# AhauBioinformatics/IDDGCN

Measured on AMD Instinct MI355X. Metric: adjacency edges/s per IDDGCN training step (pos fwd + neg fwd + bwd + Adam), higher is better.
Workload: dtype f32

## Files before the change

### iddgcn_amd/csrc/iddgcn_hip.hip

```cpp
#include <hip/hip_runtime.h>
#include <stdint.h>

#include <type_traits>

#include "../../include/iddgcn.h"

typedef float f32x4 __attribute__((ext_vector_type(4)));
typedef float f32x16 __attribute__((ext_vector_type(16)));
typedef _Float16 f16x4 __attribute__((ext_vector_type(4)));
typedef _Float16 f16x8 __attribute__((ext_vector_type(8)));
typedef __bf16 bf16x8 __attribute__((ext_vector_type(8)));
typedef __bf16 bf16x4 __attribute__((ext_vector_type(4)));
typedef short s16x4 __attribute__((ext_vector_type(4)));
typedef unsigned int u32x2 __attribute__((ext_vector_type(2)));
typedef unsigned int u32x4 __attribute__((ext_vector_type(4)));

#define MAX_R 8
#define EPS_BCE 1e-7f

namespace {

__device__ __forceinline__ float sigmoidf_(float x) { return 1.0f / (1.0f + expf(-x)); }
__device__ __forceinline__ float sigmoid_fast(float x) { return __builtin_amdgcn_rcpf(1.0f + __expf(-x)); }

// ... 1555 lines not shown
            __builtin_amdgcn_sched_barrier(0);
        }
        __builtin_amdgcn_sched_barrier(0);
        {
            v4s16 ta[2][2], tb[2][4][2];
#pragma unroll
            for (int s = 0; s < 2; ++s) {
                const int ra = 16 * s + 8 * (lane >> 5) + xs, rq = ra + 4;
                tr_read_asm(ta[s][0], xb + ra * XPT + 16 * ((4 * wb + colq) ^ stn_sw(ra)) + cb);
                tr_read_asm(ta[s][1], xb + rq * XPT + 16 * ((4 * wb + colq) ^ stn_sw(rq)) + cb);
#pragma unroll
                for (int j = 0; j < 4; ++j) {
                    const int blk = cbase + j;
                    tr_read_asm(tb[s][j][0], dob + ra * DPT + 16 * ((4 * blk + colq) ^ stn_sw(ra)) + cb);
                    tr_read_asm(tb[s][j][1], dob + rq * DPT + 16 * ((4 * blk + colq) ^ stn_sw(rq)) + cb);
                }
            }
            asm volatile("s_waitcnt lgkmcnt(0)"
                         : "+v"(ta[0][0]), "+v"(ta[0][1]), "+v"(ta[1][0]), "+v"(ta[1][1]), "+v"(tb[0][0][0]),
                           "+v"(tb[0][0][1]), "+v"(tb[0][1][0]), "+v"(tb[0][1][1]), "+v"(tb[0][2][0]),
                           "+v"(tb[0][2][1]), "+v"(tb[0][3][0]), "+v"(tb[0][3][1]), "+v"(tb[1][0][0]),
                           "+v"(tb[1][0][1]), "+v"(tb[1][1][0]), "+v"(tb[1][1][1]), "+v"(tb[1][2][0]),
                           "+v"(tb[1][2][1]), "+v"(tb[1][3][0]), "+v"(tb[1][3][1])::"memory");
#pragma unroll
            for (int s = 0; s < 2; ++s) {
                const bf16x8 a = __builtin_bit_cast(bf16x8, __builtin_shufflevector(ta[s][0], ta[s][1], 0, 1, 2, 3, 4, 5, 6, 7));
#pragma unroll
                for (int j = 0; j < 4; ++j)
                    tacc[j] = __builtin_amdgcn_mfma_f32_32x32x16_bf16(
                        a, __builtin_bit_cast(bf16x8, __builtin_shufflevector(tb[s][j][0], tb[s][j][1], 0, 1, 2, 3, 4, 5, 6, 7)),
                        tacc[j], 0, 0, 0);
            }
        }
        __builtin_amdgcn_sched_barrier(0);
    };
    auto epilogue = [&](long long t, int bb, const f32x4 (&sacc)[2]) __attribute__((always_inline)) -> int {
        const char* xb = lds + bb * BUF + DOB;
        const long long row0 = t * TR;
        const long long left = M - row0;
        const unsigned nbytes = (unsigned)((left < TR ? left : TR) * D * 2);
        const __amdgpu_buffer_rsrc_t rc =
            __builtin_amdgcn_make_buffer_rsrc(reinterpret_cast<char*>(X) + row0 * D * 2, (short)0, nbytes, 0x00020000);
        const int xc = (2 * wave + (g >> 1)) ^ swi;
#pragma unroll
        for (int rb = 0; rb < 2; ++rb) {
            const int r = 16 * rb + i16;
            const f32x4 x = bf4_to_f32(*reinterpret_cast<const bf16x4*>(xb + r * XPT + 16 * xc + 8 * (g & 1)));
            f32x4 v = sacc[rb];
#pragma unroll
            for (int q = 0; q < 4; ++q) v[q] = v[q] * (x[q] * (1.0f - x[q]));
            __builtin_amdgcn_raw_buffer_store_b64(__builtin_bit_cast(u32x2, f32_to_bf4(v)), rc, (r * D + c0 + 4 * g) * 2,
                                                  0, 0);
        }
        return 2;
    };

    if (t_beg < t_end) {
        int dc[PD], sc[PD];
#pragma unroll
        for (int k = 0; k < PD; ++k) {
            dc[k] = t_beg + k < t_end ? stage(t_beg + k, k) : 0;
            sc[k] = 0;
        }
        int younger = 0;
#pragma unroll
        for (int k = 1; k < PD; ++k) younger += dc[k];
        wait_vm(younger);
        asm volatile("s_waitcnt lgkmcnt(0)" ::: "memory");
        __syncthreads();
        f32x4 sacc[2];
        int b = 0;
        for (long long t = t_beg; t < t_end; ++t) {
            const int it = (int)(t - t_beg);
            const int slot = it % PD;
            dc[slot] = t + PD < t_end ? stage(t + PD, (b + PD) % NBUF) : 0;
            mfma_tile(b, sacc);
            sc[slot] = epilogue(t, b, sacc);
            int y = sc[(it + 1) % PD];
#pragma unroll
            for (int j = 2; j <= PD; ++j) {
                const int s2 = (it + j) % PD;
                y += dc[s2] + sc[s2];
            }
            wait_vm(y);
            asm volatile("s_waitcnt lgkmcnt(0)" ::: "memory");
            __builtin_amdgcn_s_barrier();
            asm volatile("" ::: "memory");
            b = (b + 1) % NBUF;
        }
    }
    float* out = slab + (long long)range * D * D;
    const int i = lane & 31, h = lane >> 5;
#pragma unroll
    for (int j = 0; j < 4; ++j)
#pragma unroll
        for (int k = 0; k < 16; ++k) {
            const int row = 128 * half + 32 * wb + (k & 3) + 8 * (k >> 2) + 4 * h;
            out[row * D + 32 * (cbase + j) + i] = tacc[j][k];
        }
}

__device__ __forceinline__ void split3(float x, __bf16& b0, __bf16& b1, __bf16& b2) {
    b0 = (__bf16)x;
    const float r1 = x - (float)b0;
    b1 = (__bf16)r1;
    b2 = (__bf16)(r1 - (float)b1);
}
typedef float f32x2v __attribute__((ext_vector_type(2)));
typedef __bf16 bf16x2v __attribute__((ext_vector_type(2)));
__device__ __forceinline__ unsigned cvt_pk_bf16(float a, float b) {
    return __builtin_bit_cast(unsigned, __builtin_convertvector(f32x2v{a, b}, bf16x2v));
}
__device__ __forceinline__ void split3x2(float x0, float x1, unsigned& p0, unsigned& p1, unsigned& p2) {
    p0 = cvt_pk_bf16(x0, x1);
    const float r0 = x0 - __builtin_bit_cast(float, p0 << 16);
    const float r1 = x1 - __builtin_bit_cast(float, p0 & 0xffff0000u);
    p1 = cvt_pk_bf16(r0, r1);
    const float s0 = r0 - __builtin_bit_cast(float, p1 << 16);
    const float s1 = r1 - __builtin_bit_cast(float, p1 & 0xffff0000u);
    p2 = cvt_pk_bf16(s0, s1);
}
__device__ __forceinline__ void split3x4(const f32x4& v, bf16x4& p0, bf16x4& p1, bf16x4& p2) {
    unsigned a0, b0, c0, a1, b1, c1;
    split3x2(v[0], v[1], a0, b0, c0);
    split3x2(v[2], v[3], a1, b1, c1);
    const u32x2 a = {a0, a1}, b = {b0, b1}, c = {c0, c1};
    p0 = __builtin_bit_cast(bf16x4, a);
    p1 = __builtin_bit_cast(bf16x4, b);
    p2 = __builtin_bit_cast(bf16x4, c);
}
__device__ __forceinline__ void planes_from3(const f32x4& x, char* row, int lane) {
    bf16x4 p0, p1, p2;
    split3x4(x, p0, p1, p2);
    *reinterpret_cast<bf16x4*>(row + lane * 8) = p0;
    *reinterpret_cast<bf16x4*>(row + 512 + lane * 8) = p1;
    *reinterpret_cast<bf16x4*>(row + 1024 + lane * 8) = p2;
}
__device__ __forceinline__ void row_to_planes3(char* row, int lane) {
    planes_from3(ld4(reinterpret_cast<const float*>(row) + lane * 4), row, lane);
}

__device__ __forceinline__ unsigned lds_u32(const void* p) {
    return (unsigned)(uintptr_t)(__attribute__((address_space(3))) const char*)p;
}
namespace rb3 {
constexpr int D = 256, NW = 8, TR = 32, CWG = 128, CWV = 16;
constexpr int PITCH = 1568;
constexpr int ABYTES = TR * PITCH;
constexpr int RPW = TR / NW;
constexpr int SLAB = TR * CWV;
}
__device__ __forceinline__ int slab16_off(int slot, int g) { return slot * 16 + 4 * (g ^ ((-(slot >> 2)) & 3)); }

template <int NV, bool AUX, bool BC = false>
__global__ __launch_bounds__(512) void rowgemm256_b3_kernel(RowGemmP p, int n_ranges) {
    using namespace rb3;
    static_assert(NV >= 0 && NV <= 2 && !(NV > 0 && AUX), "b3: gathered forward (NV = R = 1, 2), sigma' backward, plain");
    static_assert(!BC || NV == 0, "BC: one broadcast V row per relation (R <= 2), e.g. dz W_a^T");
    constexpr int NSL = NV + (AUX ? 1 : 0);
    constexpr int WF = NSL * SLAB + 64 + 64 + 32;
    constexpr int LDSB = 2 * ABYTES + NW * WF * 4;
    static_assert(LDSB <= 160 * 1024, "LDS budget");
    __shared__ __attribute__((aligned(16))) char lds[LDSB];
    const int lane = threadIdx.x & 63;
    const int wave = __builtin_amdgcn_readfirstlane(threadIdx.x >> 6);
    const int i = lane & 15, g = lane >> 4;
    const int bx = blockIdx.x;
    const int half = (bx >> 3) & 1;
    const int range = ((bx >> 4) << 3) | (bx & 7);
    if (range >= n_ranges) return;
    const int c0 = half * CWG + wave * CWV;
    float* slabw = reinterpret_cast<float*>(lds + 2 * ABYTES) + wave * WF;
    float* coefw = slabw + NSL * SLAB;
    int* idxw = reinterpret_cast<int*>(coefw + 64);
    int* cmpw = idxw + 64;

    const long long ntiles = ((long long)p.M + TR - 1) / TR;
    const long long t_beg = (long long)range * p.tiles_per_block;
    long long t_end = t_beg + p.tiles_per_block;
    if (t_end > ntiles) t_end = ntiles;
    if (t_beg >= t_end) return;
    const long long Mlast = (long long)p.M - 1;
    auto clampe = [&](long long e) __attribute__((always_inline)) { return e > Mlast ? Mlast : e; };

    bf16x8 w0[8], w1[8], w2[8];
#pragma unroll
    for (int q = 0; q < 8; ++q)
#pragma unroll
        for (int e = 0; e < 8; ++e) {
            const int k = 32 * q + 8 * g + e;
            const float wv = p.b_trans ? p.B[(c0 + i) * D + k] : p.B[k * D + c0 + i];
            __bf16 a, b, c;
            split3(wv, a, b, c);
            w0[q][e] = a;
            w1[q][e] = b;
            w2[q][e] = c;
        }

    f32x4 vb[2] = {f32x4{0.f, 0.f, 0.f, 0.f}, f32x4{0.f, 0.f, 0.f, 0.f}};
    if constexpr (BC) {
#pragma unroll
        for (int r = 0; r < 2; ++r)
            if (r < p.R) vb[r] = ld4(p.V + r * p.v_rel_stride + c0 + 4 * g);
    }
    auto dma_idx = [&](long long t) __attribute__((always_inline)) -> int {
        if (NV == 0 || !p.v_idx || t >= t_end) return 0;
        const int* src = p.v_idx + (lane < 32 ? clampe(t * TR + lane) : 0);
        __builtin_amdgcn_global_load_lds((gbl_vptr)src, (lds_vptr)idxw, 4, 0, 0);
        return 1;
    };
    auto dma_A = [&](long long t, int bb) __attribute__((always_inline)) -> int {
        if (t >= t_end) return 0;
#pragma unroll
        for (int j = 0; j < RPW; ++j) {
            const int r = wave * RPW + j;
            const float* src = p.A + clampe(t * TR + r) * D + lane * 4;
            __builtin_amdgcn_global_load_lds((gbl_vptr)src, (lds_vptr)(lds + bb * ABYTES + r * PITCH), 16, 0, 0);
        }
        return RPW;
    };
    auto convert = [&](int bb) __attribute__((always_inline)) {
#pragma unroll
        for (int j = 0; j < RPW; ++j) row_to_planes3(lds + bb * ABYTES + (wave * RPW + j) * PITCH, lane);
    };
    int vs0 = 0, vs1 = 0;
    auto dma_slabs = [&](long long t) __attribute__((always_inline)) -> int {
        int n = 0;
        if constexpr (NV > 0) {
            int vi = 0;
            bool start = false;
            if (lane < 32) {
                const long long e = clampe(t * TR + lane);
                vi = p.v_idx ? idxw[lane] : (int)e;
                const int prev = p.v_idx ? idxw[lane > 0 ? lane - 1 : 0] : (int)e - 1;
                start = lane == 0 || vi != prev;
            }
            const unsigned long long m = __ballot(start);
            const int u = __popcll(m);
            vs0 = __popcll(m & ((2ull << i) - 1)) - 1;
            vs1 = __popcll(m & ((2ull << (16 + i)) - 1)) - 1;
            if (start) cmpw[__popcll(m & ((2ull << lane) - 1)) - 1] = vi;
            asm volatile("s_waitcnt lgkmcnt(0)" ::: "memory");
            for (int kb = 0; kb < u; kb += 16) {
                const int slot = kb + (lane >> 2);
                const int gg = (lane & 3) ^ ((-(slot >> 2)) & 3);
                const long long v = cmpw[slot < u ? slot : u - 1];
#pragma unroll
                for (int r = 0; r < NV; ++r) {
                    const float* src = p.V + r * p.v_rel_stride + v * D + c0 + gg * 4;
                    __builtin_amdgcn_global_load_lds((gbl_vptr)src, (lds_vptr)(slabw + r * SLAB + kb * 16), 16, 0, 0);
                }
                n += NV;
            }
            const long long last = (long long)p.M * NV - 1;
            long long ci = t * TR * NV + lane;
            if (ci > last) ci = last;
            __builtin_amdgcn_global_load_lds((gbl_vptr)(p.coef + ci), (lds_vptr)coefw, 4, 0, 0);
            n += 1;
        }
        if constexpr (BC) {
            const long long last = (long long)p.M * p.R - 1;
            long long ci = t * TR * p.R + lane;
            if (ci > last) ci = last;
            __builtin_amdgcn_global_load_lds((gbl_vptr)(p.coef + ci), (lds_vptr)coefw, 4, 0, 0);
            n += 1;
        }
        if constexpr (AUX) {
#pragma unroll
            for (int k = 0; k < 2; ++k) {
                const int slot = 16 * k + (lane >> 2);
                const int gg = (lane & 3) ^ ((-(slot >> 2)) & 3);
                const float* src = p.aux + clampe(t * TR + slot) * D + c0 + gg * 4;
                __builtin_amdgcn_global_load_lds((gbl_vptr)src, (lds_vptr)(slabw + NV * SLAB + k * 256), 16, 0, 0);
            }
            n += 2;
        }
        return n;
    };
    auto epilogue = [&](long long t, const f32x4 (&acc)[2]) __attribute__((always_inline)) -> int {
        const long long row0 = t * TR;
        const long long left = (long long)p.M - row0;
        const unsigned nbytes = (unsigned)((left < TR ? left : TR) * D * 4);
        const __amdgpu_buffer_rsrc_t rc =
            __builtin_amdgcn_make_buffer_rsrc(reinterpret_cast<char*>(p.C) + row0 * D * 4, (short)0, nbytes, 0x00020000);
#pragma unroll
        for (int rh = 0; rh < 2; ++rh) {
            const int row = 16 * rh + i;
            f32x4 v = acc[rh];
            if constexpr (NV > 0) {
                const int vs = rh ? vs1 : vs0;
#pragma unroll
                for (int r = 0; r < NV; ++r) {
                    const float cf = coefw[row * NV + r];
                    const f32x4 s = ld4(slabw + r * SLAB + slab16_off(vs, g));
#pragma unroll
                    for (int q = 0; q < 4; ++q) v[q] = fmaf(cf, s[q], v[q]);
                }
            }
            if constexpr (BC) {
#pragma unroll
                for (int r = 0; r < 2; ++r) {
                    if (r >= p.R) break;
                    const float cf = coefw[row * p.R + r];
#pragma unroll
                    for (int q = 0; q < 4; ++q) v[q] = fmaf(cf, vb[r][q], v[q]);
                }
            }
            if (AUX && p.accumulate) {
                v += ld4(slabw + NV * SLAB + slab16_off(row, g));
            } else if (p.act == IDDGCN_ACT_SIGMOID) {
#pragma unroll
                for (int q = 0; q < 4; ++q) v[q] = sigmoid_fast(v[q]);
            } else if (AUX && p.act == IDDGCN_ACT_DSIGMOID) {
                const f32x4 x = ld4(slabw + NV * SLAB + slab16_off(row, g));
#pragma unroll
                for (int q = 0; q < 4; ++q) v[q] = v[q] * (x[q] * (1.0f - x[q]));
            }
            __builtin_amdgcn_raw_buffer_store_b128(v, rc, (row * D + c0 + 4 * g) * 4, 0, 0);
        }
        return 2;
    };
    auto mfma_tile = [&](int bb, f32x4 (&acc)[2]) __attribute__((always_inline)) {
        f32x4 hi0 = {0.f, 0.f, 0.f, 0.f}, lo0 = hi0, hi1 = hi0, lo1 = hi0;
        const unsigned ab = (unsigned)(uintptr_t)(__attribute__((address_space(3))) char*)(lds + bb * ABYTES) +
                            i * PITCH + 16 * g;
        u32x4 fx[2][3], fy[2][3];
        asm volatile("s_waitcnt lgkmcnt(0)" ::: "memory");
#define B3_LOADQ(Q, S)                                                                                    \
        asm volatile("ds_read_b128 %0, %6 offset:%7\n\tds_read_b128 %1, %6 offset:%8\n\t"                 \
                     "ds_read_b128 %2, %6 offset:%9\n\tds_read_b128 %3, %6 offset:%10\n\t"                \
                     "ds_read_b128 %4, %6 offset:%11\n\tds_read_b128 %5, %6 offset:%12"                   \
                     : "=&v"(fx[S][0]), "=&v"(fx[S][1]), "=&v"(fx[S][2]), "=&v"(fy[S][0]), "=&v"(fy[S][1]),     \
                       "=&v"(fy[S][2])                                                                   \
                     : "v"(ab), "i"(64 * (Q)), "i"(64 * (Q) + 512), "i"(64 * (Q) + 1024),                \
                       "i"(64 * (Q) + 16 * PITCH), "i"(64 * (Q) + 16 * PITCH + 512),                      \
                       "i"(64 * (Q) + 16 * PITCH + 1024)                                                 \
                     : "memory")
        B3_LOADQ(0, 0);
#pragma unroll
        for (int q = 0; q < 8; ++q) {
            const int S = q & 1;
            if (q + 1 < 8) {
                switch (q) {
                    case 0: B3_LOADQ(1, 1); break;
                    case 1: B3_LOADQ(2, 0); break;
                    case 2: B3_LOADQ(3, 1); break;
                    case 3: B3_LOADQ(4, 0); break;
                    case 4: B3_LOADQ(5, 1); break;
                    case 5: B3_LOADQ(6, 0); break;
                    default: B3_LOADQ(7, 1); break;
                }
                asm volatile("s_waitcnt lgkmcnt(6)"
                             : "+v"(fx[S][0]), "+v"(fx[S][1]), "+v"(fx[S][2]), "+v"(fy[S][0]), "+v"(fy[S][1]),
                               "+v"(fy[S][2])::"memory");
            } else {
                asm volatile("s_waitcnt lgkmcnt(0)"
                             : "+v"(fx[S][0]), "+v"(fx[S][1]), "+v"(fx[S][2]), "+v"(fy[S][0]), "+v"(fy[S][1]),
                               "+v"(fy[S][2])::"memory");
            }
            const bf16x8 x0 = __builtin_bit_cast(bf16x8, fx[S][0]), x1 = __builtin_bit_cast(bf16x8, fx[S][1]),
                         x2 = __builtin_bit_cast(bf16x8, fx[S][2]);
            const bf16x8 y0 = __builtin_bit_cast(bf16x8, fy[S][0]), y1 = __builtin_bit_cast(bf16x8, fy[S][1]),
                         y2 = __builtin_bit_cast(bf16x8, fy[S][2]);
            lo0 = __builtin_amdgcn_mfma_f32_16x16x32_bf16(w0[q], x2, lo0, 0, 0, 0);
            lo1 = __builtin_amdgcn_mfma_f32_16x16x32_bf16(w0[q], y2, lo1, 0, 0, 0);
            lo0 = __builtin_amdgcn_mfma_f32_16x16x32_bf16(w2[q], x0, lo0, 0, 0, 0);
            lo1 = __builtin_amdgcn_mfma_f32_16x16x32_bf16(w2[q], y0, lo1, 0, 0, 0);
            lo0 = __builtin_amdgcn_mfma_f32_16x16x32_bf16(w1[q], x1, lo0, 0, 0, 0);
            lo1 = __builtin_amdgcn_mfma_f32_16x16x32_bf16(w1[q], y1, lo1, 0, 0, 0);
            lo0 = __builtin_amdgcn_mfma_f32_16x16x32_bf16(w0[q], x1, lo0, 0, 0, 0);
            lo1 = __builtin_amdgcn_mfma_f32_16x16x32_bf16(w0[q], y1, lo1, 0, 0, 0);
            lo0 = __builtin_amdgcn_mfma_f32_16x16x32_bf16(w1[q], x0, lo0, 0, 0, 0);
            lo1 = __builtin_amdgcn_mfma_f32_16x16x32_bf16(w1[q], y0, lo1, 0, 0, 0);
            hi0 = __builtin_amdgcn_mfma_f32_16x16x32_bf16(w0[q], x0, hi0, 0, 0, 0);
            hi1 = __builtin_amdgcn_mfma_f32_16x16x32_bf16(w0[q], y0, hi1, 0, 0, 0);
        }
#undef B3_LOADQ
        acc[0] = hi0 + lo0;
        acc[1] = hi1 + lo1;
    };

    dma_idx(t_beg);
    asm volatile("s_waitcnt vmcnt(0)" ::: "memory");
    dma_A(t_beg, 0);
    dma_slabs(t_beg);
    asm volatile("s_waitcnt vmcnt(0) lgkmcnt(0)" ::: "memory");
    convert(0);
    dma_idx(t_beg + 1);
    asm volatile("s_waitcnt vmcnt(0) lgkmcnt(0)" ::: "memory");
    __syncthreads();

#define B3_MAIN_LOOP(LATE)                                                                           \
    {                                                                                                \
        f32x4 acc[2];                                                                                \
        int b = 0;                                                                                   \
        for (long long t = t_beg; t < t_end; ++t) {                                                  \
            const bool more = t + 1 < t_end;                                                         \
            const int nA = dma_A(t + 1, b ^ 1);                                                      \
            int after_A = 0;                                            \
            if (LATE && t > t_beg) {                                                                 \
                wait_vm(nA);                                                 \
                after_A += epilogue(t - 1, acc);                                                     \
                asm volatile("s_waitcnt lgkmcnt(0)" ::: "memory");                                   \
                after_A += dma_slabs(t);                                                             \
                asm volatile("s_waitcnt lgkmcnt(0)" ::: "memory");                                   \
                after_A += dma_idx(t + 1);                                                           \
            }                                                                                        \
            mfma_tile(b, acc);                                                                       \
            if (LATE) {                                                                              \
                if (more) {                                                                          \
                    wait_vm(after_A);                                                                \
                    convert(b ^ 1);                                                                  \
                }                                                                                    \
            } else {                                                                                 \
                wait_vm(nA);                                                 \
                after_A += epilogue(t, acc);                                                         \
                if (more) {                                                                          \
                    wait_vm(after_A);                                                    \
                    convert(b ^ 1);                                                                  \
                    asm volatile("s_waitcnt lgkmcnt(0)" ::: "memory");                               \
                    dma_slabs(t + 1);                                                                \
                    asm volatile("s_waitcnt lgkmcnt(0)" ::: "memory");                               \
                    dma_idx(t + 2);                                                                  \
                }                                                                                    \
            }                                                                                        \
            asm volatile("s_waitcnt lgkmcnt(0)" ::: "memory");                                       \
            __builtin_amdgcn_s_barrier();                                                            \
            asm volatile("" ::: "memory");                                                           \
            b ^= 1;                                                                                  \
        }                                                                                            \
        if (LATE) {                                                                                  \
            asm volatile("s_waitcnt vmcnt(0)" ::: "memory");                                         \
            epilogue(t_end - 1, acc);                                                                \
        }                                                                                            \
    }
    if (wave >= 4) B3_MAIN_LOOP(true) else B3_MAIN_LOOP(false)
#undef B3_MAIN_LOOP
}

namespace tb3 {
constexpr int D = 256, TK = 16, PT = 1600, OPB = TK * PT, BUF = 2 * OPB, NBUF = 3;
}
__device__ __forceinline__ bf16x8 tr_frag_b3(const char* p0) {
    typedef __attribute__((address_space(3))) v4s16* l4p;
    const v4s16 a = __builtin_amdgcn_ds_read_tr16_b64_v4i16((l4p)p0);
    const v4s16 b = __builtin_amdgcn_ds_read_tr16_b64_v4i16((l4p)(p0 + 4 * tb3::PT));
    return __builtin_bit_cast(bf16x8, __builtin_shufflevector(a, b, 0, 1, 2, 3, 4, 5, 6, 7));
}
__global__ __launch_bounds__(512) void gemm_tn256_b3_kernel(long long M_, long long rpb_, const float* __restrict__ A_,
                                                            const float* __restrict__ B_, float* __restrict__ slab_,
                                                            TnBatch tb) {
    using namespace tb3;
    const bool bat = tb.n > 0;
    const int ent = bat ? (int)blockIdx.y : 0;
    if (bat && (int)blockIdx.x >= tb.nb[ent]) return;
    const long long M = bat ? tb.M[ent] : M_;
    const long long rows_per_block = bat ? tb.rpb[ent] : rpb_;
    const float* __restrict__ A = bat ? tb.A[ent] : A_;
    const float* __restrict__ B = bat ? tb.B[ent] : B_;
    float* __restrict__ slab = bat ? tb.slab[ent] : slab_;
    static_assert(NBUF * BUF <= 160 * 1024, "LDS budget");
    __shared__ __attribute__((aligned(16))) char lds[NBUF * BUF];
    const int lane = threadIdx.x & 63;
    const int wave = __builtin_amdgcn_readfirstlane(threadIdx.x >> 6);
    const bool late = wave >= 4;
    f32x16 acc[8];
#pragma unroll
    for (int cj = 0; cj < 8; ++cj)
#pragma unroll
        for (int j = 0; j < 16; ++j) acc[cj][j] = 0.f;
    const long long r_beg = (long long)blockIdx.x * rows_per_block;
    long long r_end = r_beg + rows_per_block;
    if (r_end > M) r_end = M;
    const long long nt = r_end > r_beg ? (r_end - r_beg + TK - 1) / TK : 0;

    auto stage = [&](long long t, int bb) __attribute__((always_inline)) {
        int n = 0;
#pragma unroll
        for (int j = 0; j < 2; ++j) {
            const int r = 2 * wave + j;
            const long long e = r_beg + t * TK + r;
            char* ra = lds + bb * BUF + r * PT;
            if (e < r_end) {
                __builtin_amdgcn_global_load_lds((gbl_vptr)(A + e * D + lane * 4), (lds_vptr)ra, 16, 0, 0);
                __builtin_amdgcn_global_load_lds((gbl_vptr)(B + e * D + lane * 4), (lds_vptr)(ra + OPB), 16, 0, 0);
                n += 2;
            } else {
                st4(reinterpret_cast<float*>(ra) + lane * 4, f32x4{0.f, 0.f, 0.f, 0.f});
                st4(reinterpret_cast<float*>(ra + OPB) + lane * 4, f32x4{0.f, 0.f, 0.f, 0.f});
            }
        }
        return n;
    };
    auto convert = [&](int bb) __attribute__((always_inline)) {
#pragma unroll
        for (int j = 0; j < 2; ++j) {
            char* ra = lds + bb * BUF + (2 * wave + j) * PT;
            row_to_planes3(ra, lane);
            row_to_planes3(ra + OPB, lane);
        }
    };
    auto wait_newest = [&](int n) __attribute__((always_inline)) {
        if (n >= 4) asm volatile("s_waitcnt vmcnt(4)" ::: "memory");
        else if (n >= 2) asm volatile("s_waitcnt vmcnt(2)" ::: "memory");
        else asm volatile("s_waitcnt vmcnt(0)" ::: "memory");
    };
    const int roff = (8 * (lane >> 5) + ((lane >> 2) & 3)) * PT + 2 * (16 * ((lane >> 4) & 1) + 4 * (lane & 3));
    auto tie6 = [&](v4s16 (&f)[3][2]) __attribute__((always_inline)) {
        asm volatile("s_waitcnt lgkmcnt(0)"
                     : "+v"(f[0][0]), "+v"(f[0][1]), "+v"(f[1][0]), "+v"(f[1][1]), "+v"(f[2][0]), "+v"(f[2][1])::"memory");
    };
    auto frag = [&](const v4s16 (&f)[2]) __attribute__((always_inline)) {
        return __builtin_bit_cast(bf16x8, __builtin_shufflevector(f[0], f[1], 0, 1, 2, 3, 4, 5, 6, 7));
    };
    auto mfma_tile = [&](int bb) __attribute__((always_inline)) {
        const char* pa = lds + bb * BUF + roff + 64 * wave;
        const char* pb0 = lds + bb * BUF + OPB + roff;
        v4s16 fa[3][2], fb[3][2], fn[3][2];
#pragma unroll
        for (int k = 0; k < 3; ++k) {
            tr_read_asm(fa[k][0], pa + 512 * k);
            tr_read_asm(fa[k][1], pa + 512 * k + 4 * PT);
            tr_read_asm(fb[k][0], pb0 + 512 * k);
            tr_read_asm(fb[k][1], pb0 + 512 * k + 4 * PT);
        }
        tie6(fa);
        tie6(fb);
        const bf16x8 a0 = frag(fa[0]), a1 = frag(fa[1]), a2 = frag(fa[2]);
#pragma unroll
        for (int cj = 0; cj < 8; ++cj) {
            if (cj + 1 < 8) {
                const char* pb = pb0 + 64 * (cj + 1);
#pragma unroll
// ... 1514 lines not shown
    if (i < n) {
#pragma unroll 8
        for (int b = b0; b < b1; ++b) s += slab[(long long)b * n + i];
    }
    part[w][lane] = s;
    __syncthreads();
    if (w == 0 && i < n) {
        float t = part[0][lane];
#pragma unroll
        for (int q = 1; q < 16; ++q) t += part[q][lane];
        t *= scale;
        out[i] = accumulate ? out[i] + t : t;
    }
}
void launch_reduce_slabs(hipStream_t st, int n_slabs, long long n, const float* slab, float* out, int accumulate,
                         float scale) {
    const bool few_blocks = n / 4 < 64 * 64 && n_slabs >= 64;
    if (n % 4 == 0 && n_slabs >= 8 && !few_blocks && (reinterpret_cast<uintptr_t>(slab) & 15) == 0) {
        const long long n4 = n / 4;
        hipLaunchKernelGGL(reduce_slabs4_kernel, dim3((unsigned)((n4 + 63) / 64)), dim3(256), 0, st, n_slabs, n4,
                           reinterpret_cast<const f32x4*>(slab), out, accumulate, scale);
    } else if (n_slabs >= 64) {
        hipLaunchKernelGGL(reduce_slabs_split_kernel, dim3((unsigned)((n + 63) / 64)), dim3(1024), 0, st, n_slabs, n,
                           slab, out, accumulate, scale);
    } else {
        hipLaunchKernelGGL(reduce_slabs_kernel, dim3((unsigned)((n + 255) / 256)), dim3(256), 0, st, n_slabs, n, slab,
                           out, accumulate, scale);
    }
}

__global__ __launch_bounds__(256) void adam_kernel(long long n, float* __restrict__ var, float* __restrict__ m,
                                                   float* __restrict__ v, const float* __restrict__ g, float alpha,
                                                   float b1, float b2, float eps, int sparse_form,
                                                   const float* __restrict__ alpha_table,
                                                   const int* __restrict__ step) {
    const long long i = (long long)blockIdx.x * blockDim.x + threadIdx.x;
    if (i >= n) return;
    if (alpha_table) alpha = alpha_table[*step];
    const float gi = g[i];
    float mi = m[i], vi = v[i];
    if (sparse_form) {
        mi = mi * b1 + gi * (1.0f - b1);
        vi = vi * b2 + (gi * gi) * (1.0f - b2);
    } else {
        mi = mi + (gi - mi) * (1.0f - b1);
        vi = vi + (gi * gi - vi) * (1.0f - b2);
    }
    m[i] = mi;
    v[i] = vi;
    var[i] = var[i] - (mi * alpha) / (sqrtf(vi) + eps);
}

__global__ void step_advance_kernel(int* __restrict__ step, float* __restrict__ loss_history,
                                    const float* __restrict__ loss) {
    if (threadIdx.x != 0) return;
    const int s = *step;
    if (loss_history && loss) loss_history[s] = *loss;
    *step = s + 1;
}

struct V3Sel {
    int nv;
    bool aux, hc;
    bool cw = false;
    bool pl = false;
    bool split = false;
    bool c4 = false;
    bool same(const V3Sel& o) const {
        return nv == o.nv && aux == o.aux && hc == o.hc && cw == o.cw && pl == o.pl && split == o.split &&
               c4 == o.c4;
    }
};
bool v3_select(const RowGemmP& p, V3Sel& sel) {
    const bool gatherV = p.R > 0 && p.v_row_stride != 0;
    const bool dsig = p.act == IDDGCN_ACT_DSIGMOID;
    if (gatherV) {
        if (dsig || p.v_row_stride != 256) return false;
        sel = {p.R <= 2 ? p.R : (p.R <= 4 ? 4 : 8), false, true};
    } else {
        sel = {0, dsig, p.R > 0, p.R > 2};
    }
    sel.split = p.precision == IDDGCN_GEMM_SPLIT_F16;
    sel.c4 = p.precision == IDDGCN_GEMM_F32_4CHAIN;
    if (sel.c4 && (sel.nv || sel.aux || sel.hc)) return false;
    sel.pl = (p.planes & (IDDGCN_PLANES_C | IDDGCN_PLANES_AUX)) != 0;
    if (!sel.pl) return true;
    if ((p.planes & IDDGCN_PLANES_C) && !(sel.nv >= 1 && sel.nv <= 2 && !sel.aux)) return false;
    if ((p.planes & IDDGCN_PLANES_AUX) && !(sel.aux && sel.nv == 0 && !sel.hc)) return false;
    return true;
}

RowGemmP to_p(const iddgcn_rowgemm_t& a) {
    RowGemmP p;
    p.M = a.M; p.A = a.A; p.a_idx = a.a_idx; p.B = a.B; p.b_trans = a.b_trans;
    p.C = a.C; p.accumulate = a.accumulate; p.R = a.R; p.coef = a.coef; p.coef_idx = a.coef_idx;
    p.V = a.V; p.v_idx = a.v_idx; p.v_rel_stride = a.v_rel_stride; p.v_row_stride = a.v_row_stride;
    p.act = a.act; p.aux = a.aux; p.planes = a.planes; p.precision = a.precision;
    p.tiles_per_block = 1;
    return p;
}
int check_rowgemm(const iddgcn_rowgemm_t& a) {
    if (!dim_ok(a.D)) return IDDGCN_E_BAD_DIM;
    if (a.R < 0 || a.R > MAX_R) return IDDGCN_E_BAD_REL;
    if (a.precision != IDDGCN_GEMM_EXACT_F32 && a.precision != IDDGCN_GEMM_SPLIT_F16 &&
        a.precision != IDDGCN_GEMM_F32_4CHAIN && a.precision != IDDGCN_GEMM_BF16X3)
        return IDDGCN_E_BAD_ARG;
    if (a.precision == IDDGCN_GEMM_F32_4CHAIN && a.D == 256 && (a.R > 0 || a.act == IDDGCN_ACT_DSIGMOID || a.planes))
        return IDDGCN_E_BAD_ARG;
    if (a.M == 0) return 0;
    if (a.M < 0 || !a.A || !a.B || !a.C) return IDDGCN_E_BAD_ARG;
    if (a.R > 0 && (!a.coef || !a.V)) return IDDGCN_E_BAD_ARG;
    if (a.act == IDDGCN_ACT_DSIGMOID && !a.aux) return IDDGCN_E_BAD_ARG;
    if (a.act < IDDGCN_ACT_NONE || a.act > IDDGCN_ACT_DSIGMOID) return IDDGCN_E_BAD_ARG;
    if (a.planes) {
        if (a.planes & ~(IDDGCN_PLANES_A | IDDGCN_PLANES_C | IDDGCN_PLANES_AUX)) return IDDGCN_E_BAD_ARG;
        if (a.D != 256 || a.precision != IDDGCN_GEMM_SPLIT_F16 || a.a_idx) return IDDGCN_E_BAD_ARG;
        if ((a.planes & IDDGCN_PLANES_C) && (a.act != IDDGCN_ACT_SIGMOID || a.accumulate)) return IDDGCN_E_BAD_ARG;
        if ((a.planes & IDDGCN_PLANES_AUX) && a.act != IDDGCN_ACT_DSIGMOID) return IDDGCN_E_BAD_ARG;
        V3Sel sel;
        if (!v3_select(to_p(a), sel)) return IDDGCN_E_BAD_ARG;
    }
    return 0;
}

bool b3_select(const RowGemmP& p, int& nv, bool& aux, bool& bc) {
    bc = false;
    if (p.precision != IDDGCN_GEMM_BF16X3 || p.a_idx || p.planes) return false;
    if (p.R > 0 && p.v_row_stride == 0 && !p.v_idx) {
        if (p.R > 2 || p.coef_idx || p.accumulate || p.act == IDDGCN_ACT_SIGMOID) return false;
        nv = 0;
        aux = p.act == IDDGCN_ACT_DSIGMOID;
        bc = true;
        return true;
    }
    if (p.R > 0) {
        if (p.R > 2 || p.v_row_stride != 256 || p.coef_idx || p.act == IDDGCN_ACT_DSIGMOID || p.accumulate) return false;
        nv = p.R;
        aux = false;
        return true;
    }
    if (p.accumulate && p.act != IDDGCN_ACT_NONE) return false;
    nv = 0;
    aux = p.act == IDDGCN_ACT_DSIGMOID || p.accumulate;
    return true;
}
void launch_b3(hipStream_t st, RowGemmP p, int nv, bool aux, bool bc) {
    const long long nt = ((long long)p.M + rb3::TR - 1) / rb3::TR;
    long long nr = nt < 128 ? nt : 128;
    p.tiles_per_block = (int)((nt + nr - 1) / nr);
    nr = (nt + p.tiles_per_block - 1) / p.tiles_per_block;
    nr = (nr + 7) / 8 * 8;
    const int n_ranges = (int)nr;
    if (p.accumulate) p.aux = p.C;
    const dim3 g((unsigned)(2 * nr)), blk(512);
    if (bc && aux) hipLaunchKernelGGL((rowgemm256_b3_kernel<0, true, true>), g, blk, 0, st, p, n_ranges);
    else if (bc) hipLaunchKernelGGL((rowgemm256_b3_kernel<0, false, true>), g, blk, 0, st, p, n_ranges);
    else if (nv == 1) hipLaunchKernelGGL((rowgemm256_b3_kernel<1, false>), g, blk, 0, st, p, n_ranges);
    else if (nv == 2) hipLaunchKernelGGL((rowgemm256_b3_kernel<2, false>), g, blk, 0, st, p, n_ranges);
    else if (aux) hipLaunchKernelGGL((rowgemm256_b3_kernel<0, true>), g, blk, 0, st, p, n_ranges);
    else hipLaunchKernelGGL((rowgemm256_b3_kernel<0, false>), g, blk, 0, st, p, n_ranges);
}

void launch_v3(hipStream_t st, RowGemmBatch& pb, int n, const V3Sel& sel, bool bf = false) {
    const long long per = n > 0 ? (256 / n > 0 ? 256 / n : 1) : 256;
    long long nbmax = 0;
    for (int k = 0; k < n; ++k) {
        RowGemmP& p = pb.p[k];
        const long long nt = ((long long)p.M + r3::TR - 1) / r3::TR;
        long long nb = nt < per ? nt : per;
        if (nb < 1) nb = 1;
        p.tiles_per_block = (int)((nt + nb - 1) / nb);
        if (p.tiles_per_block < 1) p.tiles_per_block = 1;
        nb = (nt + p.tiles_per_block - 1) / p.tiles_per_block;
        if (nb > nbmax) nbmax = nb;
    }
    if (nbmax == 0) return;
    const dim3 g((unsigned)nbmax, (unsigned)n), blk(512);
    if (bf) {
#define V3B(NV, AUX, HC)                                                                                         \
    do {                                                                                                          \
        if (pb.p[0].precision == IDDGCN_GEMM_BF16)                                                                \
            hipLaunchKernelGGL((rowgemm256_v3_kernel<NV, AUX, HC, true, false, true, false, false, true>), g, blk, 0, st, pb); \
        else hipLaunchKernelGGL((rowgemm256_v3_kernel<NV, AUX, HC, true, false, true>), g, blk, 0, st, pb);        \
    } while (0)
        if (sel.nv == 1) V3B(1, false, true);
        else if (sel.nv == 2) V3B(2, false, true);
        else if (sel.nv == 4) V3B(4, false, true);
        else if (sel.nv == 8) V3B(8, false, true);
        else if (sel.aux) V3B(0, true, false);
        else V3B(0, false, false);
#undef V3B
        return;
    }
    const bool x3 = sel.split;
#define V3L(NV, AUX, HC)                                                                        \
    {                                                                                           \
        if (x3) hipLaunchKernelGGL((rowgemm256_v3_kernel<NV, AUX, HC, true>), g, blk, 0, st, pb); \
        else hipLaunchKernelGGL((rowgemm256_v3_kernel<NV, AUX, HC, false>), g, blk, 0, st, pb);   \
    }
#define V3W(AUX)                                                                                     \
    {                                                                                                \
        if (x3) hipLaunchKernelGGL((rowgemm256_v3_kernel<0, AUX, true, true, true>), g, blk, 0, st, pb); \
        else hipLaunchKernelGGL((rowgemm256_v3_kernel<0, AUX, true, false, true>), g, blk, 0, st, pb);   \
    }
    if (sel.c4) {
        hipLaunchKernelGGL((rowgemm256_v3_kernel<0, false, false, false, false, false, false, true>), g, blk, 0, st, pb);
    } else if (sel.pl) {
        if (sel.nv == 1) hipLaunchKernelGGL((rowgemm256_v3_kernel<1, false, true, true, false, false, true>), g, blk, 0, st, pb);
        else if (sel.nv == 2) hipLaunchKernelGGL((rowgemm256_v3_kernel<2, false, true, true, false, false, true>), g, blk, 0, st, pb);
        else hipLaunchKernelGGL((rowgemm256_v3_kernel<0, true, false, true, false, false, true>), g, blk, 0, st, pb);
    } else if (sel.nv == 1) V3L(1, false, true)
    else if (sel.nv == 2) V3L(2, false, true)
    else if (sel.nv == 4) V3L(4, false, true)
    else if (sel.nv == 8) V3L(8, false, true)
    else if (sel.hc && sel.cw) {
        if (sel.aux) V3W(true)
        else V3W(false)
    } else if (sel.hc && sel.aux) V3L(0, true, true)
    else if (sel.hc) V3L(0, false, true)
    else if (sel.aux) V3L(0, true, false)
    else V3L(0, false, false)
#undef V3L
#undef V3W
}

template <bool BF, bool PL>
int run_combine_out(void* stream, int M, int d, int R, const float* Y, const int* idx, const float* coef,
                    const float* V, long long v_rel_stride, void* out) {
    if (d != 256) return IDDGCN_E_BAD_DIM;
    if (R < 0 || R > MAX_R) return IDDGCN_E_BAD_REL;
    if (M < 0 || !Y || !idx || !out || (R > 0 && (!coef || !V))) return IDDGCN_E_BAD_ARG;
    if (M == 0) return 0;
    const long long nchunk = ((long long)M + RC_CH - 1) / RC_CH;
    long long nb = (nchunk + 3) / 4;
    if (nb > 2048) nb = 2048;
    hipStream_t st = (hipStream_t)stream;
    float* o = (float*)out;
#define RCB(RR) hipLaunchKernelGGL((run_combine256_kernel<RR, BF, PL>), dim3((unsigned)nb), dim3(256), 0, st, M, Y, idx, coef, V, v_rel_stride, o)
    switch (R) {
        case 0: RCB(0); break;
        case 1: RCB(1); break;
        case 2: RCB(2); break;
        case 3: RCB(3); break;
        case 4: RCB(4); break;
        case 5: RCB(5); break;
        case 6: RCB(6); break;
        case 7: RCB(7); break;
        default: RCB(8); break;
    }
#undef RCB
    return launch_status();
}

inline unsigned grid_for(long long rows, int lpr) {
    const long long threads = rows * lpr;
    return (unsigned)((threads + 255) / 256);
}

namespace fg8 {
constexpr int D = 256, R = 8, TR = 64, NW = 8, NBUF = 3;
constexpr int RPW = TR / NW;
constexpr int PITCH = 512;
constexpr int ABUF = TR * PITCH;
constexpr int CAPS = 4;
constexpr int SLOTB = 1088;
constexpr int WIDX = 0, WTAIL = 256, WCOEF = 512, WV = WCOEF + TR * R * 4;
constexpr int WREG = WV + CAPS * SLOTB;
constexpr int LDSB = NBUF * ABUF + NW * WREG;
static_assert(LDSB <= 160 * 1024, "LDS budget");
}

template <bool HL>
__global__ __launch_bounds__(512) void fwd_gather8_bf16_kernel(RowGemmP p) {
    using namespace fg8;
    __shared__ __attribute__((aligned(16))) char lds[LDSB];
    const int lane = threadIdx.x & 63;
    const int wave = __builtin_amdgcn_readfirstlane(threadIdx.x >> 6);
    auto fresh_lane = [&]() __attribute__((always_inline)) {
        int l = lane;
        asm volatile("" : "+v"(l));
        return l;
    };
    const int i16 = lane & 15, g = lane >> 4;
    const int c0 = wave * 32;
    char* wreg = lds + NBUF * ABUF + wave * WREG;
    int* idxw = reinterpret_cast<int*>(wreg + WIDX);
    int* tailw = reinterpret_cast<int*>(wreg + WTAIL);
    float* coefw = reinterpret_cast<float*>(wreg + WCOEF);
    char* vsl = wreg + WV;
    const long long vrs = p.v_rel_stride;

    const long long ntiles = ((long long)p.M + TR - 1) / TR;
    const long long t_beg = (long long)blockIdx.x * p.tiles_per_block;
    long long t_end = t_beg + p.tiles_per_block;
    if (t_end > ntiles) t_end = ntiles;
    if (t_beg >= t_end) return;
    const long long Mlast = (long long)p.M - 1;
    auto clampe = [&](long long e) __attribute__((always_inline)) { return e > Mlast ? Mlast : e; };

    bf16x8 wh[2][8], wl[2][HL ? 8 : 1];
#pragma unroll
    for (int cb = 0; cb < 2; ++cb)
#pragma unroll
        for (int q = 0; q < 8; ++q)
#pragma unroll
            for (int j = 0; j < 8; ++j) {
                const float w = p.B[(32 * q + 8 * g + j) * D + c0 + 16 * cb + i16];
                const __bf16 hi = (__bf16)w;
                wh[cb][q][j] = hi;
                if constexpr (HL) wl[cb][q][j] = (__bf16)(w - (float)hi);
            }
// ... 999 lines not shown
```

Measured before the change: 79.37 million.

## Split K across two wave groups in gathered-forward b3 row GEMM

Adds a KS=2 variant of the b3 row-GEMM kernel that launches 1024 threads. The second group of 8 waves computes the upper half of K and hands its partial accumulators to the first group through LDS. The first group also runs the gather, slab DMA and epilogue. This halves the per-wave register footprint for weights and aims to raise MFMA concurrency for the gathered forward (NV=1,2). The cost is extra barriers per tile and an LDS reduction buffer, and the loads are no longer double-buffered inside a tile.

```diff
diff --git a/iddgcn_amd/csrc/iddgcn_hip.hip b/iddgcn_amd/csrc/iddgcn_hip.hip
--- a/iddgcn_amd/csrc/iddgcn_hip.hip
+++ b/iddgcn_amd/csrc/iddgcn_hip.hip
@@ -1731,18 +1731,24 @@
 }
 __device__ __forceinline__ int slab16_off(int slot, int g) { return slot * 16 + 4 * (g ^ ((-(slot >> 2)) & 3)); }
 
-template <int NV, bool AUX, bool BC = false>
-__global__ __launch_bounds__(512) void rowgemm256_b3_kernel(RowGemmP p, int n_ranges) {
+template <int NV, bool AUX, bool BC = false, int KS = 1>
+__global__ __launch_bounds__(512 * KS) void rowgemm256_b3_kernel(RowGemmP p, int n_ranges) {
     using namespace rb3;
     static_assert(NV >= 0 && NV <= 2 && !(NV > 0 && AUX), "b3: gathered forward (NV = R = 1, 2), sigma' backward, plain");
     static_assert(!BC || NV == 0, "BC: one broadcast V row per relation (R <= 2), e.g. dz W_a^T");
+    static_assert(KS == 1 || (KS == 2 && NV > 0), "k-split: the gathered forward only");
     constexpr int NSL = NV + (AUX ? 1 : 0);
     constexpr int WF = NSL * SLAB + 64 + 64 + 32;
-    constexpr int LDSB = 2 * ABYTES + NW * WF * 4;
+    constexpr int KQ = 8 / KS;
+    constexpr int XOFF = 2 * ABYTES + NW * WF * 4;
+    constexpr int XB = TR * CWV * 4;
+    constexpr int LDSB = XOFF + (KS == 2 ? NW * XB : 0);
     static_assert(LDSB <= 160 * 1024, "LDS budget");
     __shared__ __attribute__((aligned(16))) char lds[LDSB];
     const int lane = threadIdx.x & 63;
-    const int wave = __builtin_amdgcn_readfirstlane(threadIdx.x >> 6);
+    const int wid = __builtin_amdgcn_readfirstlane(threadIdx.x >> 6);
+    const int wave = KS == 2 ? (wid & 7) : wid;
+    const int kh = KS == 2 ? (wid >> 3) : 0;
     const int i = lane & 15, g = lane >> 4;
     const int bx = blockIdx.x;
     const int half = (bx >> 3) & 1;
@@ -1762,12 +1768,12 @@
     const long long Mlast = (long long)p.M - 1;
     auto clampe = [&](long long e) __attribute__((always_inline)) { return e > Mlast ? Mlast : e; };
 
-    bf16x8 w0[8], w1[8], w2[8];
-#pragma unroll
-    for (int q = 0; q < 8; ++q)
+    bf16x8 w0[KQ], w1[KQ], w2[KQ];
+#pragma unroll
+    for (int q = 0; q < KQ; ++q)
 #pragma unroll
         for (int e = 0; e < 8; ++e) {
-            const int k = 32 * q + 8 * g + e;
+            const int k = 32 * q + 8 * g + e + (KS == 2 ? 128 * kh : 0);
             const float wv = p.b_trans ? p.B[(c0 + i) * D + k] : p.B[k * D + c0 + i];
             __bf16 a, b, c;
             split3(wv, a, b, c);
@@ -1901,6 +1907,54 @@
     };
     auto mfma_tile = [&](int bb, f32x4 (&acc)[2]) __attribute__((always_inline)) {
         f32x4 hi0 = {0.f, 0.f, 0.f, 0.f}, lo0 = hi0, hi1 = hi0, lo1 = hi0;
+#define B3_MFMAQ(Q, X0, X1, X2, Y0, Y1, Y2)                                                              \
+        lo0 = __builtin_amdgcn_mfma_f32_16x16x32_bf16(w0[Q], X2, lo0, 0, 0, 0);                           \
+        lo1 = __builtin_amdgcn_mfma_f32_16x16x32_bf16(w0[Q], Y2, lo1, 0, 0, 0);                           \
+        lo0 = __builtin_amdgcn_mfma_f32_16x16x32_bf16(w2[Q], X0, lo0, 0, 0, 0);                           \
+        lo1 = __builtin_amdgcn_mfma_f32_16x16x32_bf16(w2[Q], Y0, lo1, 0, 0, 0);                           \
+        lo0 = __builtin_amdgcn_mfma_f32_16x16x32_bf16(w1[Q], X1, lo0, 0, 0, 0);                           \
+        lo1 = __builtin_amdgcn_mfma_f32_16x16x32_bf16(w1[Q], Y1, lo1, 0, 0, 0);                           \
+        lo0 = __builtin_amdgcn_mfma_f32_16x16x32_bf16(w0[Q], X1, lo0, 0, 0, 0);                           \
+        lo1 = __builtin_amdgcn_mfma_f32_16x16x32_bf16(w0[Q], Y1, lo1, 0, 0, 0);                           \
+        lo0 = __builtin_amdgcn_mfma_f32_16x16x32_bf16(w1[Q], X0, lo0, 0, 0, 0);                           \
+        lo1 = __builtin_amdgcn_mfma_f32_16x16x32_bf16(w1[Q], Y0, lo1, 0, 0, 0);                           \
+        hi0 = __builtin_amdgcn_mfma_f32_16x16x32_bf16(w0[Q], X0, hi0, 0, 0, 0);                           \
+        hi1 = __builtin_amdgcn_mfma_f32_16x16x32_bf16(w0[Q], Y0, hi1, 0, 0, 0)
+        if constexpr (KS == 2) {
+            const unsigned ab = (unsigned)(uintptr_t)(__attribute__((address_space(3))) char*)(lds + bb * ABYTES) +
+                                i * PITCH + 16 * g + 256 * kh;
+            u32x4 fx[3], fy[3];
+            asm volatile("s_waitcnt lgkmcnt(0)" ::: "memory");
+#define B3_LOADQ1(Q)                                                                                     \
+            asm volatile("ds_read_b128 %0, %6 offset:%7\n\tds_read_b128 %1, %6 offset:%8\n\t"             \
+                         "ds_read_b128 %2, %6 offset:%9\n\tds_read_b128 %3, %6 offset:%10\n\t"            \
+                         "ds_read_b128 %4, %6 offset:%11\n\tds_read_b128 %5, %6 offset:%12"               \
+                         : "=&v"(fx[0]), "=&v"(fx[1]), "=&v"(fx[2]), "=&v"(fy[0]), "=&v"(fy[1]), "=&v"(fy[2]) \
+                         : "v"(ab), "i"(64 * (Q)), "i"(64 * (Q) + 512), "i"(64 * (Q) + 1024),            \
+                           "i"(64 * (Q) + 16 * PITCH), "i"(64 * (Q) + 16 * PITCH + 512),                  \
+                           "i"(64 * (Q) + 16 * PITCH + 1024)                                             \
+                         : "memory")
+#pragma unroll
+            for (int q = 0; q < KQ; ++q) {
+                switch (q) {
+                    case 0: B3_LOADQ1(0); break;
+                    case 1: B3_LOADQ1(1); break;
+                    case 2: B3_LOADQ1(2); break;
+                    default: B3_LOADQ1(3); break;
+                }
+                asm volatile("s_waitcnt lgkmcnt(0)"
+                             : "+v"(fx[0]), "+v"(fx[1]), "+v"(fx[2]), "+v"(fy[0]), "+v"(fy[1]), "+v"(fy[2])::"memory");
+                const bf16x8 x0 = __builtin_bit_cast(bf16x8, fx[0]), x1 = __builtin_bit_cast(bf16x8, fx[1]),
+                             x2 = __builtin_bit_cast(bf16x8, fx[2]);
+                const bf16x8 y0 = __builtin_bit_cast(bf16x8, fy[0]), y1 = __builtin_bit_cast(bf16x8, fy[1]),
+                             y2 = __builtin_bit_cast(bf16x8, fy[2]);
+                B3_MFMAQ(q, x0, x1, x2, y0, y1, y2);
+            }
+#undef B3_LOADQ1
+            acc[0] = hi0 + lo0;
+            acc[1] = hi1 + lo1;
+            return;
+        }
         const unsigned ab = (unsigned)(uintptr_t)(__attribute__((address_space(3))) char*)(lds + bb * ABYTES) +
                             i * PITCH + 16 * g;
         u32x4 fx[2][3], fy[2][3];
@@ -1917,7 +1971,7 @@
                      : "memory")
         B3_LOADQ(0, 0);
 #pragma unroll
-        for (int q = 0; q < 8; ++q) {
+        for (int q = 0; q < KQ; ++q) {
             const int S = q & 1;
             if (q + 1 < 8) {
                 switch (q) {
@@ -1955,9 +2009,70 @@
             hi1 = __builtin_amdgcn_mfma_f32_16x16x32_bf16(w0[q], y0, hi1, 0, 0, 0);
         }
 #undef B3_LOADQ
+#undef B3_MFMAQ
         acc[0] = hi0 + lo0;
         acc[1] = hi1 + lo1;
     };
+
+    if constexpr (KS == 2) {
+        f32x4* xw = reinterpret_cast<f32x4*>(lds + XOFF + wave * XB) + lane;
+        f32x4 acc[2];
+        int b = 0;
+        if (kh) {
+            dma_A(t_beg, 0);
+            asm volatile("s_waitcnt vmcnt(0)" ::: "memory");
+            convert(0);
+            asm volatile("s_waitcnt lgkmcnt(0)" ::: "memory");
+            __syncthreads();
+            for (long long t = t_beg; t < t_end; ++t) {
+                const int nA = dma_A(t + 1, b ^ 1);
+                mfma_tile(b, acc);
+                if (nA) {
+                    asm volatile("s_waitcnt vmcnt(0)" ::: "memory");
+                    convert(b ^ 1);
+                }
+                __builtin_amdgcn_s_barrier();
+                asm volatile("" ::: "memory");
+                xw[0] = acc[0];
+                xw[64] = acc[1];
+                asm volatile("s_waitcnt lgkmcnt(0)" ::: "memory");
+                __builtin_amdgcn_s_barrier();
+                asm volatile("" ::: "memory");
+                b ^= 1;
+            }
+        } else {
+            dma_idx(t_beg);
+            asm volatile("s_waitcnt vmcnt(0)" ::: "memory");
+            dma_slabs(t_beg);
+            asm volatile("s_waitcnt lgkmcnt(0)" ::: "memory");
+            dma_idx(t_beg + 1);
+            __syncthreads();
+            for (long long t = t_beg; t < t_end; ++t) {
+                if (t > t_beg) {
+                    asm volatile("s_waitcnt vmcnt(0)" ::: "memory");
+                    acc[0] = acc[0] + xw[0];
+                    acc[1] = acc[1] + xw[64];
+                    epilogue(t - 1, acc);
+                    asm volatile("s_waitcnt lgkmcnt(0)" ::: "memory");
+                    dma_slabs(t);
+                    asm volatile("s_waitcnt lgkmcnt(0)" ::: "memory");
+                    dma_idx(t + 1);
+                }
+                mfma_tile(b, acc);
+                asm volatile("s_waitcnt lgkmcnt(0)" ::: "memory");
+                __builtin_amdgcn_s_barrier();
+                asm volatile("" ::: "memory");
+                __builtin_amdgcn_s_barrier();
+                asm volatile("" ::: "memory");
+                b ^= 1;
+            }
+            asm volatile("s_waitcnt vmcnt(0)" ::: "memory");
+            acc[0] = acc[0] + xw[0];
+            acc[1] = acc[1] + xw[64];
+            epilogue(t_end - 1, acc);
+        }
+        return;
+    }
 
     dma_idx(t_beg);
     asm volatile("s_waitcnt vmcnt(0)" ::: "memory");
@@ -3778,11 +3893,11 @@
     nr = (nr + 7) / 8 * 8;
     const int n_ranges = (int)nr;
     if (p.accumulate) p.aux = p.C;
-    const dim3 g((unsigned)(2 * nr)), blk(512);
+    const dim3 g((unsigned)(2 * nr)), blk(512), blk2(1024);
     if (bc && aux) hipLaunchKernelGGL((rowgemm256_b3_kernel<0, true, true>), g, blk, 0, st, p, n_ranges);
     else if (bc) hipLaunchKernelGGL((rowgemm256_b3_kernel<0, false, true>), g, blk, 0, st, p, n_ranges);
-    else if (nv == 1) hipLaunchKernelGGL((rowgemm256_b3_kernel<1, false>), g, blk, 0, st, p, n_ranges);
-    else if (nv == 2) hipLaunchKernelGGL((rowgemm256_b3_kernel<2, false>), g, blk, 0, st, p, n_ranges);
+    else if (nv == 1) hipLaunchKernelGGL((rowgemm256_b3_kernel<1, false, false, 2>), g, blk2, 0, st, p, n_ranges);
+    else if (nv == 2) hipLaunchKernelGGL((rowgemm256_b3_kernel<2, false, false, 2>), g, blk2, 0, st, p, n_ranges);
     else if (aux) hipLaunchKernelGGL((rowgemm256_b3_kernel<0, true>), g, blk, 0, st, p, n_ranges);
     else hipLaunchKernelGGL((rowgemm256_b3_kernel<0, false>), g, blk, 0, st, p, n_ranges);
 }
```

Result: faster. 80.84 million, median of 6 (+1.9%).
